# Napoliee/Expressive-FastSpeech2-Mandarin

Measured on AMD Instinct MI355X. Metric: mel-frames/sec/GPU (batch-64 synth) at 1/2/4/8 MI355X; RTF, higher is better.
Workload: dtype bf16; 1 GPU; cfg2: batch=64 x 64 phonemes per GPU, ESD-Chinese-Singing-MFA model.yaml, FastSpeech2.forward eval bf16; global_batch=64, seq_len=64, mel_frames_per_gpu_batch=24883, T_max=430, parallelism=dp1 (independent shards, no collective), hip_graph=True

## Files before the change

expressive-fastspeech2-mandarin_amd/csrc/wconv.hip:

```cpp
#include <type_traits>
#include <utility>

#include "conv_common.h"
#include "fs2_common.h"

namespace {

constexpr int kUnitB = 4096;

struct WconvArgs {
  const bf16 *x;
  int64_t xs;
  const bf16 *w;
  const float *bias;
  bf16 *out;
  int64_t os;
  int B, T, M, pad;
  uint32_t x_bytes, w_bytes;
  const int2 *row_pos;
  const int32_t *rows_dev;
  int out_sc1;
  const bf16 *w2;
  const float *bias2;
  const float *res;
  int64_t rs;
  float *out2;
  int64_t os2;
// ... 372 lines not shown
#pragma unroll 2
  for (int i = tid; i < BM * CPR; i += NT) {
    const int m = i / CPR, ch = i - m * CPR;
    if (m0 + m < M)
      store16_out(ob, (uint32_t)(m0 + m) * orow + (uint32_t)ch * 16u,
                  *reinterpret_cast<const uint4 *>(smem + X_OFF + m * OPITCH + ch * 16), p.out_sc1);
  }
  }
}


struct PnHeadArgs {
  const bf16 *x;
  int64_t xs;
  const bf16 *w1, *w2;
  const float *b1, *b2;
  bf16 *out;
  int64_t os;
  int T, M, pad;
  uint32_t x_bytes, w1_bytes, w2_bytes;
  const int2 *row_pos;
  const int32_t *rows_dev;
  int out_sc1;
};

__global__ __launch_bounds__(512, 1) void pn_head_kernel(PnHeadArgs p) {
  constexpr int KS = 5, CIN1 = 80, NCOL = 512, MB = 7, BM = 112, NWV = 8, NT = 512, JB = 4, DEPTH = 4;
  constexpr int YR = BM + KS - 1;
  constexpr int XR = BM + 2 * (KS - 1);
  constexpr int YPITCH = NCOL * 2 + 32;
  constexpr int XPITCH = CIN1 * 2 + 16;
  constexpr int OPITCH = NCOL * 2 + 16;
  constexpr int XPIECES = (XR * XPITCH + 1023) / 1024;
  constexpr int XPW = (XPIECES + NWV - 1) / NWV;
  constexpr int NU1 = (KS * CIN1 + 31) / 32;
  constexpr int NKS = NCOL / 32;
  constexpr int NU2 = KS * NKS;
  constexpr int ZBYTES = NKS * 64;
  constexpr int Y_OFF = ZBYTES;
  constexpr int YREG = YR * YPITCH > BM * OPITCH ? YR * YPITCH : BM * OPITCH;
  constexpr int X_OFF = Y_OFF + YREG;
  constexpr int B1_OFF = X_OFF + NWV * XPW * 1024;
  constexpr int B2_OFF = B1_OFF + NCOL * 4;
  constexpr int SMEM = B2_OFF + NCOL * 4;
  static_assert(SMEM <= 163840, "LDS");
  __shared__ __attribute__((aligned(16))) char smem[SMEM];

  const int tid = threadIdx.x, lane = tid & 63;
  const int w = __builtin_amdgcn_readfirstlane(tid >> 6);
  const int M = p.rows_dev != nullptr ? min(*p.rows_dev, p.M) : p.M, T = p.T, pad = p.pad;
  const int m0 = blockIdx.x * BM;
  if (m0 >= M) return;
  const int hrow0 = lane & 15, hi = lane >> 4;
  auto taps = [&](int gm) {
    int v = 0;
    if (gm >= 0 && gm < M) {
      int tpos, tlen;
      seq_pos(p.row_pos, gm, T, tpos, tlen);
#pragma unroll
      for (int tap = 0; tap < KS; ++tap) v |= ((unsigned)(tpos + tap - pad) < (unsigned)tlen ? 1 : 0) << tap;
    }
    return v;
  };
  for (int i = tid; i < ZBYTES / 16; i += NT) *reinterpret_cast<float4 *>(smem + 16 * i) = make_float4(0.f, 0.f, 0.f, 0.f);
  if (w < 4)
    __builtin_amdgcn_raw_ptr_buffer_load_lds(make_rsrc(w < 2 ? p.b1 : p.b2, NCOL * 4),
                                             (__attribute__((address_space(3))) void *)(smem + B1_OFF + w * 1024), 16,
                                             (uint32_t)((w & 1) * 1024 + lane * 16), 0, 0, 0);

  const rsrc_t xr = make_rsrc(p.x, p.x_bytes);
  const rsrc_t w1r = make_rsrc(p.w1, p.w1_bytes), w2r = make_rsrc(p.w2, p.w2_bytes);
  const uint32_t xrow = (uint32_t)p.xs * 2u;
#pragma unroll
  for (int i = 0; i < XPW; ++i) {
    const int pc = w + NWV * i;
    const int o = pc * 1024 + lane * 16;
    const int r = o / XPITCH, within = o - r * XPITCH;
    const int gm = m0 - 2 * pad + r;
    const bool ok = r < XR && within < CIN1 * 2 && gm >= 0 && gm < M;
    __builtin_amdgcn_raw_ptr_buffer_load_lds(xr, (__attribute__((address_space(3))) void *)(smem + X_OFF + pc * 1024),
                                             16, ok ? (uint32_t)gm * xrow + (uint32_t)within : kOOB, 0, 0, 0);
  }

  const uint32_t lane_off = (uint32_t)lane * 16u;
  const uint32_t wb1 = (uint32_t)(w * NU1) * (uint32_t)kUnitB, wb2 = (uint32_t)(w * NU2) * (uint32_t)kUnitB;
  bf16x8 pa[DEPTH][JB];
  auto load_at = [&](auto S, int u) {
    constexpr int s = decltype(S)::value;
    const bool c1 = u < 2 * NU1;
    const int uu = c1 ? (u < NU1 ? u : u - NU1) : (u - 2 * NU1 < NU2 ? u - 2 * NU1 : 0);
    const rsrc_t r = c1 ? w1r : w2r;
    const uint32_t so = (c1 ? wb1 : wb2) + (uint32_t)uu * (uint32_t)kUnitB;
    __builtin_amdgcn_sched_barrier(0);
#pragma unroll
    for (int jb = 0; jb < JB; ++jb)
      pa[s][jb] = __builtin_bit_cast(bf16x8, __builtin_amdgcn_raw_buffer_load_b128(r, lane_off + jb * 1024, so, 0));
    __builtin_amdgcn_sched_barrier(0);
  };
  static_for<DEPTH>([&](auto S) { load_at(S, decltype(S)::value); });
  asm volatile("s_waitcnt vmcnt(%0)" ::"n"(4 * DEPTH) : "memory");
  __builtin_amdgcn_s_waitcnt(kLgkm0);
  __syncthreads();

  static_for<2>([&](auto PASS) {
    constexpr int ps = decltype(PASS)::value;
    int vm1[4];
#pragma unroll
    for (int mb = 0; mb < 4; ++mb) vm1[mb] = taps(m0 - pad + (4 * ps + mb) * 16 + hrow0);
    f32x4 acc[JB][4];
#pragma unroll
    for (int i = 0; i < JB; ++i)
#pragma unroll
      for (int j = 0; j < 4; ++j) acc[i][j] = f32x4{0.f, 0.f, 0.f, 0.f};
    auto bases = [&](int u, int (&ad)[4]) {
      const int k = 32 * u + 8 * hi;
      const int tap = k / CIN1, c = k - tap * CIN1;
      const int base = X_OFF + ((4 * ps) * 16 + hrow0 + tap) * XPITCH + c * 2;
#pragma unroll
      for (int mb = 0; mb < 4; ++mb)
        ad[mb] = tap < KS ? (base + mb * 16 * XPITCH) & __builtin_amdgcn_sbfe(vm1[mb], tap, 1) : 0;
    };
    bf16x8 f0[4], f1[4];
    auto rd = [&](const int (&ad)[4], bf16x8 (&f)[4]) {
#pragma unroll
      for (int mb = 0; mb < 4; ++mb) f[mb] = *reinterpret_cast<const bf16x8 *>(smem + ad[mb]);
// ... 17 lines not shown
#pragma unroll
    for (int jb = 0; jb < JB; ++jb) {
      const int n = w * 64 + jb * 16 + 4 * hi;
      const float4 bb = *reinterpret_cast<const float4 *>(smem + B1_OFF + 4 * n);
#pragma unroll
      for (int mb = 0; mb < 4; ++mb) {
        const int r = (4 * ps + mb) * 16 + hrow0;
        const f32x4 v = acc[jb][mb];
        bf16x4 o;
        o[0] = (bf16)tanh_fast(v[0] + bb.x);
        o[1] = (bf16)tanh_fast(v[1] + bb.y);
        o[2] = (bf16)tanh_fast(v[2] + bb.z);
        o[3] = (bf16)tanh_fast(v[3] + bb.w);
        if (r < YR) *reinterpret_cast<bf16x4 *>(smem + Y_OFF + r * YPITCH + n * 2) = o;
      }
    }
  });
  __builtin_amdgcn_s_waitcnt(kLgkm0);
  __syncthreads();

  int vm2[MB];
#pragma unroll
  for (int mb = 0; mb < MB; ++mb) vm2[mb] = taps(m0 + mb * 16 + hrow0);
  auto bases_x = [&](int tap, int (&ad)[MB]) {
    const int base = Y_OFF + (hrow0 + tap) * YPITCH + hi * 16;
#pragma unroll
    for (int mb = 0; mb < MB; ++mb) ad[mb] = (base + mb * 16 * YPITCH) & __builtin_amdgcn_sbfe(vm2[mb], tap, 1);
  };
  bf16x8 f0[MB], f1[MB];
  auto issue_x = [&](const int (&ad)[MB], auto KSI, bf16x8 (&f)[MB]) {
    constexpr int off = decltype(KSI)::value * 64;
#pragma unroll
    for (int mb = 0; mb < MB; ++mb) f[mb] = *reinterpret_cast<const bf16x8 *>(smem + ad[mb] + off);
  };
  f32x4 acc[JB][MB];
#pragma unroll
  for (int i = 0; i < JB; ++i)
#pragma unroll
    for (int j = 0; j < MB; ++j) acc[i][j] = f32x4{0.f, 0.f, 0.f, 0.f};
  auto mma = [&](const bf16x8 (&fa)[JB], const bf16x8 (&fb)[MB]) {
#pragma unroll
    for (int mb = 0; mb < MB; ++mb)
#pragma unroll
      for (int jb = 0; jb < JB; ++jb)
        acc[jb][mb] = __builtin_amdgcn_mfma_f32_16x16x32_bf16(fa[jb], fb[mb], acc[jb][mb], 0, 0, 0);
  };
  constexpr int S0 = 2 * NU1;
  int bxc[MB], bxn[MB];
  bases_x(0, bxc);
  issue_x(bxc, std::integral_constant<int, 0>{}, f0);
#pragma nounroll
  for (int tap = 0; tap < KS; ++tap) {
    bases_x(tap + 1, bxn);
    static_for<NKS>([&](auto KSI) {
      constexpr int ks = decltype(KSI)::value, sl = (S0 + ks) % DEPTH;
      if constexpr (ks + 1 < NKS) {
        if constexpr (ks & 1)
          issue_x(bxc, std::integral_constant<int, ks + 1>{}, f0);
        else
          issue_x(bxc, std::integral_constant<int, ks + 1>{}, f1);
      } else {
        issue_x(bxn, std::integral_constant<int, 0>{}, f0);
      }
      if constexpr (ks & 1)
        mma(pa[sl], f1);
      else
        mma(pa[sl], f0);
      load_at(std::integral_constant<int, sl>{}, S0 + tap * NKS + ks + DEPTH);
    });
#pragma unroll
    for (int mb = 0; mb < MB; ++mb) bxc[mb] = bxn[mb];
  }

  asm volatile("s_waitcnt vmcnt(0)" ::: "memory");
  __builtin_amdgcn_s_waitcnt(kLgkm0);
  __syncthreads();
#pragma unroll
  for (int nb = 0; nb < JB; ++nb) {
    const int n = w * 64 + nb * 16 + 4 * hi;
    const float4 bb = *reinterpret_cast<const float4 *>(smem + B2_OFF + 4 * n);
#pragma unroll
    for (int mb = 0; mb < MB; ++mb) {
      const f32x4 v = acc[nb][mb];
      bf16x4 o;
      o[0] = (bf16)tanh_fast(v[0] + bb.x);
      o[1] = (bf16)tanh_fast(v[1] + bb.y);
      o[2] = (bf16)tanh_fast(v[2] + bb.z);
      o[3] = (bf16)tanh_fast(v[3] + bb.w);
      *reinterpret_cast<bf16x4 *>(smem + Y_OFF + (hrow0 + mb * 16) * OPITCH + n * 2) = o;
    }
  }
  __syncthreads();
  constexpr int CPR = NCOL * 2 / 16;
  char *ob = reinterpret_cast<char *>(p.out);
  const uint32_t orow = (uint32_t)p.os * 2u;
#pragma unroll 2
  for (int i = tid; i < BM * CPR; i += NT) {
    const int m = i / CPR, ch = i - m * CPR;
    if (m0 + m < M)
      store16_out(ob, (uint32_t)(m0 + m) * orow + (uint32_t)ch * 16u,
                  *reinterpret_cast<const uint4 *>(smem + Y_OFF + m * OPITCH + ch * 16), p.out_sc1);
  }
}


struct PnTailArgs {
  const bf16 *x;
  int64_t xs;
  const bf16 *w;
  const float *bias;
  const float *res;
  int64_t rs;
  float *out;
  int64_t os;
  int T, M, pad;
  uint32_t x_bytes, w_bytes;
  const int2 *row_pos;
  const int32_t *rows_dev;
};

__global__ __launch_bounds__(256, 1) void pn_tail_kernel(PnTailArgs p) {
  constexpr int KS = 5, CIN = 512, NB = 5, NCOL = 80, BM = 112, NST = 3, KPS = 2;
  constexpr int XR = BM + KS - 1;
// ... 221 lines not shown
    p.w2_bytes = (uint32_t)(fs2_wconv_weight_elems(5, 512, 80) * 2);
    hipLaunchKernelGGL((wconv_kernel<5, 512, 1, true>), dim3((unsigned)((Mg + 107) / 108)), dim3(512), 0,
                       as_stream(stream), p);
  } else if (d->w2 != nullptr) {
    if (d->Cin != 80 || d->bias2 == nullptr || d->pad != 2) return FS2_EUNSUPPORTED;
    PnHeadArgs q;
    q.x = p.x;
    q.xs = p.xs;
    q.w1 = p.w;
    q.w2 = reinterpret_cast<const bf16 *>(d->w2);
    q.b1 = d->bias;
    q.b2 = d->bias2;
    q.out = p.out;
    q.os = p.os;
    q.T = p.T;
    q.M = p.M;
    q.pad = p.pad;
    q.x_bytes = p.x_bytes;
    q.w1_bytes = p.w_bytes;
    q.w2_bytes = (uint32_t)(fs2_wconv_weight_elems(d->KS, 512, 512) * 2);
    q.row_pos = row_pos;
    q.rows_dev = d->rows_dev;
    q.out_sc1 = env_out_sc1();
    hipLaunchKernelGGL(pn_head_kernel, dim3(nwg), dim3(512), 0, as_stream(stream), q);
  } else if (d->Cin == 80)
    hipLaunchKernelGGL((wconv_kernel<5, 80, 1>), dim3(nwg), dim3(512), 0, as_stream(stream), p);
  else
    hipLaunchKernelGGL((wconv_kernel<5, 512, WCONV_WQ>), dim3(nwg), dim3(512 / WCONV_WQ), 0, as_stream(stream), p);
  FS2_CHECK_LAUNCH();
  return FS2_OK;
}
```

expressive-fastspeech2-mandarin_amd/fs2amd/_lib.py:

```python
import ctypes
import os

import torch

HERE = os.path.dirname(os.path.abspath(__file__))
DEFAULT_LIB = os.path.join(HERE, "_lib", "libfs2hip.so")

FS2_F32, FS2_BF16, FS2_FP8 = 0, 1, 2
FS2_I16 = 3
FS2_F64 = 4
PITCH_T_MAX, PITCH_T_MAX_NOFILL, OUTLIER_LDS_BYTES = 131072, 4096, 65536
F0_GROUP, F0_LDS_BYTES = 8, 65536
RESAMPLE_LDS_BYTES = 81920
MAS_LDS_BYTES, MAS_LDS_SMALL, FORWARD_SUM_LDS_BYTES = 163840, 32768, 65536
MAS_AUTO, MAS_LDS, MAS_GLOBAL = 0, 1, 2
ALIGN_SIZE_CAP = 1 << 24
DTW_LDS_BYTES, DTW_LDS_SMALL = 163840, 32768
DTW_AUTO, DTW_LDS, DTW_GLOBAL = 0, 1, 2
EVAL_SIZE_CAP = 1 << 24
F0_TRACK_THR, F0_TRACK_CAP_MAX, F0_TRACK_BINS_MAX, F0_TRACK_STEP_MAX, F0_TRACK_TB = 100, 101, 256, 63, 64
F0_TRACK_LDS_BYTES = 65536
VAD_SUMS_BYTES, VAD_AREA_BYTES, VAD_TILE_FRAMES, VAD_CHUNK_FRAMES, VAD_B_MAX = 32768, 32768, 192, 256, 65535
PVOC_BLOCK, PVOC_J_CAP, PVOC_B_MAX = 64, 2 ** 31 - 1, 65535
IIR_BLOCK, IIR_CHUNK, IIR_S_MAX, IIR_TABLE_LEN, IIR_B_MAX, LOUD_H_MAX = 64, 16384, 8, 412, 65535, 32768
# ... 63 lines not shown
        ("group_n", _i), ("group_cin", _i),
    ]


class Ffn8Desc(ctypes.Structure):

    _fields_ = [
        ("x8", _p), ("x8_row_stride", _i64), ("res", _p), ("res_row_stride", _i64), ("w", _p),
        ("cs1", _p), ("b1", _p), ("inv_sf", _f), ("cs2", _p), ("b2", _p),
        ("B", _i), ("T", _i), ("D", _i), ("F", _i), ("KS", _i), ("pad", _i),
        ("ln_gamma", _p), ("ln_beta", _p), ("ln_eps", _f),
        ("out", _p), ("out_row_stride", _i64), ("out8", _p), ("out8_row_stride", _i64), ("out8_scale", _f),
        ("rows_dev", _p), ("row_pos", _p), ("rows_max", _i),
    ]


class WconvDesc(ctypes.Structure):

    _fields_ = [
        ("x", _p), ("x_row_stride", _i64), ("w", _p), ("bias", _p),
        ("B", _i), ("T", _i), ("Cin", _i), ("N", _i), ("KS", _i), ("pad", _i), ("epilogue", _i),
        ("out", _p), ("out_row_stride", _i64), ("w2", _p), ("bias2", _p), ("residual", _p), ("res_row_stride", _i64),
        ("rows_dev", _p), ("row_pos", _p), ("rows_max", _i),
    ]


class CondDesc(ctypes.Structure):

    _fields_ = [
        ("speakers", _p), ("speaker_table", _p), ("n_speaker", _i), ("emotions", _p), ("emo_table", _p),
        ("n_emo", _i), ("d_emo", _i), ("arousals", _p), ("aro_table", _p), ("n_aro", _i), ("d_aro", _i),
        ("valences", _p), ("val_table", _p), ("n_val", _i), ("d_val", _i), ("lin_w", _p), ("lin_b", _p),
        ("spk_out", _p), ("emo_out", _p),
    ]


class CondGrads(ctypes.Structure):

    _fields_ = [("d_speaker_table", _p), ("d_emo_table", _p), ("d_aro_table", _p), ("d_val_table", _p),
                ("d_lin_w", _p), ("d_lin_b", _p)]


class FfnDesc(ctypes.Structure):

    _fields_ = [
        ("x", _p), ("x_row_stride", _i64),
# ... 282 lines not shown
    "fs2_f0_track_lds_bytes": (_i64, [_i, _i]),
    "fs2_f0_track_workspace_bytes": (_i64, [_i, _i, _i, _i, _i]),
    "fs2_f0_track": (_i, [_p, _p, _i, _i, _i, _d, _i, _i, _d, _d, _p, _p, _p, _p, _p, _i, _p, _p, _i, _d, _d, _p, _i64,
                          _p, _p, _p, _p]),
}


SIGNATURES_VAD = {
    "fs2_vad_frames": (_i64, [_i64, _i64]),
    "fs2_vad_workspace_bytes": (_i64, [_i64, _i64, _i64, _i64]),
    "fs2_vad_lds_bytes": (_i64, [_i64, _i64]),
    "fs2_vad_power": (_i, [_p, _i, _i64, _p, _i, _i, _i, _i, _p, _p, _p, _i64, _p]),
    "fs2_vad_intervals": (_i, [_p, _p, _p, _i, _i, _i, _d, _d, _i, _i64, _i, _i, _p, _p, _p, _p, _p]),
    "fs2_vad_cut": (_i, [_p, _i, _i64, _p, _i, _i, _i, _p, _p, _p]),
}


SIGNATURES_PVOC = {
    "fs2_pvoc_frames": (_i64, [_i64, _d]),
    "fs2_phase_vocoder": (_i, [ctypes.POINTER(PvocDesc), _p]),
}


SIGNATURES_IIR = {
    "fs2_iir_blocks": (_i64, [_i64]),
    "fs2_iir_chunks": (_i64, [_i64]),
    "fs2_loudness_blocks": (_i64, [_i64, _i64]),
    "fs2_loudness_workspace_bytes": (_i64, [_i64, _i64, _i64]),
    "fs2_sosfilt": (_i, [_p, _i, _i64, _p, _i, _i, _p, _p, _i, _p, _p, _p, _p, _p]),
    "fs2_loudness_gate": (_i, [_p, _p, _i, _i, _i, _d, _d, _p, _p, _p, _i64, _p]),
    "fs2_gain_int16": (_i, [_p, _i, _i64, _p, _i, _i, _p, _d, _d, _p, _p, _p, _p, _p, _p]),
}


def iir_blocks(n):
    return 0 if n < 1 else (n - 1) // IIR_BLOCK + 1


def iir_chunks(n):
    return 0 if n < 1 else (n - 1) // IIR_CHUNK + 1


def loudness_blocks(n, H):
    return 0 if n < 1 or n < 4 * H else (n - 4 * H) // H + 1


# ... 121 lines not shown

def header_symbols(header_path):
    import re

    text = open(header_path).read()
    return sorted(set(re.findall(r"\b(fs2_[a-z0-9_]+)\s*\(", text)) - {"fs2_conv_desc"})


_LIB = None
CSRC = os.path.join(os.path.dirname(HERE), "csrc")
HEADER = os.path.join(os.path.dirname(os.path.dirname(HERE)), "include", "fs2hip.h")
HEADER_PROSODY = os.path.join(os.path.dirname(HEADER), "fs2hip_prosody.h")
HEADER_AUDIO = os.path.join(os.path.dirname(HEADER), "fs2hip_audio.h")
HEADER_AUDIO_INV = os.path.join(os.path.dirname(HEADER), "fs2hip_audio_inv.h")
HEADER_PREP = os.path.join(os.path.dirname(HEADER), "fs2hip_prep.h")
HEADER_F0 = os.path.join(os.path.dirname(HEADER), "fs2hip_f0.h")
HEADER_RESAMPLE = os.path.join(os.path.dirname(HEADER), "fs2hip_resample.h")
HEADER_ALIGN = os.path.join(os.path.dirname(HEADER), "fs2hip_align.h")
HEADER_EVAL = os.path.join(os.path.dirname(HEADER), "fs2hip_eval.h")
HEADER_F0_TRACK = os.path.join(os.path.dirname(HEADER), "fs2hip_f0_track.h")
HEADER_VAD = os.path.join(os.path.dirname(HEADER), "fs2hip_vad.h")
HEADER_PVOC = os.path.join(os.path.dirname(HEADER), "fs2hip_pvoc.h")
HEADER_IIR = os.path.join(os.path.dirname(HEADER), "fs2hip_iir.h")
EXTRA_HEADERS = ("fs2hip_prosody.h", "fs2hip_audio.h", "fs2hip_audio_inv.h", "fs2hip_prep.h", "fs2hip_f0.h",
                 "fs2hip_resample.h", "fs2hip_align.h", "fs2hip_eval.h", "fs2hip_f0_track.h", "fs2hip_vad.h",
                 "fs2hip_pvoc.h", "fs2hip_iir.h")


def source_build_id(csrc=CSRC, header=HEADER):
    import hashlib

    if not os.path.isdir(csrc) or not os.path.exists(header):
        return None
    h = hashlib.sha256()
    for name in sorted(f for f in os.listdir(csrc) if f.endswith((".hip", ".h"))):
        h.update(name.encode())
        with open(os.path.join(csrc, name), "rb") as f:
            h.update(f.read())
    with open(header, "rb") as f:
        h.update(b"fs2hip.h")
        h.update(f.read())
    for name in EXTRA_HEADERS:
        with open(os.path.join(os.path.dirname(header), name), "rb") as f:
            h.update(name.encode())
            h.update(f.read())
    return h.hexdigest()[:16]


def lib_path():
    return os.environ.get("FS2_LIB", DEFAULT_LIB)


def load():
    global _LIB
    if _LIB is not None:
        return _LIB
    path = lib_path()
    if not os.path.exists(path):
        raise RuntimeError(
            f"fs2amd: HIP library not found at {path}. Build it with `python -c 'import __graft_entry__ as g; "
            f"g.build()'` (hipcc --offload-arch=gfx950). There is no CPU fallback.")
    lib = ctypes.CDLL(path, mode=ctypes.RTLD_GLOBAL)
    allow_missing = "FS2_LIB" in os.environ and os.environ.get("FS2_LIB_ALLOW_MISSING") == "1"
    for name, (res, args) in list(SIGNATURES.items()) + list(SIGNATURES_PROSODY.items()) + \
            list(SIGNATURES_AUDIO.items()) + list(SIGNATURES_AUDIO_INV.items()) + list(SIGNATURES_PREP.items()) + \
            list(SIGNATURES_F0.items()) + list(SIGNATURES_RESAMPLE.items()) + list(SIGNATURES_ALIGN.items()) + \
            list(SIGNATURES_EVAL.items()) + list(SIGNATURES_F0_TRACK.items()) + list(SIGNATURES_VAD.items()) + \
            list(SIGNATURES_PVOC.items()) + list(SIGNATURES_IIR.items()):
        if allow_missing and not hasattr(lib, name):
            continue
        fn = getattr(lib, name)
        fn.restype = res
        fn.argtypes = args
    if "FS2_LIB" not in os.environ:
        want = source_build_id()
        got = lib.fs2_build_id().decode()
        if want is not None and got != want:
            raise RuntimeError(f"fs2amd: {path} was built from other sources (fs2_build_id {got}, sources "
                               f"{want}); rebuild with `python -c 'import __graft_entry__ as g; g.build()'`")
    _LIB = lib
    return lib


def check(rc, what):
    if rc != FS2_OK:
        msg = load().fs2_status_string(rc).decode()
        raise RuntimeError(f"{what} failed: fs2 status {rc} ({msg})")
```

expressive-fastspeech2-mandarin_amd/fs2amd/ops.py:

```python
import collections
import ctypes
import os

import torch

from . import _lib as L

_lib = L.load()


def _ptr(t):
    return None if t is None else ctypes.c_void_p(t.data_ptr())


def _stream(t):
    return ctypes.c_void_p(torch.cuda.current_stream(t.device).cuda_stream)


def _dt(t):
    if t.dtype == torch.bfloat16:
        return L.FS2_BF16
    if t.dtype == torch.float32:
        return L.FS2_F32
    if t.dtype == torch.float8_e4m3fn:
# ... 409 lines not shown
            out = torch.empty(*rs, 80, device=x.device, dtype=torch.float32)
        d = L.WconvDesc()
        _wconv_layout(d, layout)
        d.x, d.x_row_stride = x.data_ptr(), _rows(x, "x")
        d.w, d.bias = w_packed.data_ptr(), bias.data_ptr()
        d.B, d.T, d.Cin, d.N, d.KS, d.pad, d.epilogue = B, T, cin, N, ks, pad, L.EPI_BIAS_TANH
        d.out, d.out_row_stride = out.data_ptr(), _rows(out, "out")
        d.w2, d.bias2 = wt.data_ptr(), bt.data_ptr()
        d.residual, d.res_row_stride = res.data_ptr(), _rows(res, "residual")
        L.check(_lib.fs2_wconv(ctypes.byref(d), _stream(x)), "fs2_wconv")
        return out
    if out is None:
        out = torch.empty(*rs, N, device=x.device, dtype=torch.bfloat16)
    d = L.WconvDesc()
    _wconv_layout(d, layout)
    d.x, d.x_row_stride = x.data_ptr(), _rows(x, "x")
    d.w, d.bias = w_packed.data_ptr(), bias.data_ptr()
    d.B, d.T, d.Cin, d.N, d.KS, d.pad, d.epilogue = B, T, cin, N, ks, pad, L.EPI_BIAS_TANH
    d.out, d.out_row_stride = out.data_ptr(), _rows(out, "out")
    if second is not None:
        d.w2, d.bias2 = second[0].data_ptr(), second[1].data_ptr()
    L.check(_lib.fs2_wconv(ctypes.byref(d), _stream(x)), "fs2_wconv")
    return out


FFN_SLOTS = 256


def ffn_part_bytes(tile_rows):
    return 4 * 4 * (tile_rows // 16) * 64 * 16


def rows_bucket(rows, capacity, step=1024):
    return min(capacity, -(-int(rows) // step) * step)


FFN_COST = {112: (20.0, 10.0, {1: 0.0, 2: 10.0, 4: 16.0}), 96: (17.5, 8.5, {2: 10.0}),
            64: (13.0, 5.0, {1: 0.0, 2: 9.0, 4: 21.0})}


def ffn_form(rows, F):
    nch = F // 256
    if not _splitk_on[0]:
        return 112, 1
    best = None
    for tr, (chunk, base, over) in FFN_COST.items():
# ... 1989 lines not shown
```

expressive-fastspeech2-mandarin_amd/fs2amd/runtime.py:

```python
import os
from types import SimpleNamespace

import numpy as np
import torch

from . import _lib as L
from . import ops
from .model import sinusoid_table


def _mask(lengths, width):
    if lengths.is_cuda:
        return ops.length_mask(lengths, width)
    ids = torch.arange(0, width, device=lengths.device).unsqueeze(0).expand(lengths.shape[0], -1)
    return ids >= lengths.unsqueeze(1).expand(-1, width)


def _pe(P, which, n):
    tab = P.enc_pe if which == "enc" else P.dec_pe
    if n <= tab.shape[0]:
        return tab
    key = f"_pe_{which}_{n}"
    if not hasattr(P, key):
        setattr(P, key, sinusoid_table(n, tab.shape[1]).to(tab.device))
# ... 468 lines not shown
    dec_lens = st.mel_len if g.d_targets is None else g.mel_lens
    frame_level = not (st.phoneme_p and st.phoneme_e)
    x = st.x
    if not frame_level and T_dec == T_out and packed_decoder_ok(P):
        x, lay = decode_packed(P, st, x, dec_lens, T_out, rows_hint)
        mel, pn = mel_postnet(P, x, lay, dec_lens, postnet_valid, rows_hint)
        return mel, pn, st
    _ensure_lr(st)
    if frame_level:
        x = ops.lr_expand(x, st.cum, st.mel_len, T_out, pe=None, out_dtype=P.act_dtype)
        if not st.phoneme_p:
            st.p_pred = _variance(P, "pitch", x, dec_lens, g.p_targets, p_control)
        if not st.phoneme_e:
            st.e_pred = _variance(P, "energy", x, dec_lens, g.e_targets, e_control)
        x = x[:, :T_dec].contiguous()
        x = _add_pe(x, _pe(P, "dec", T_dec))
    else:
        x = ops.lr_expand(x, st.cum, st.mel_len, T_out, pe=_pe(P, "dec", T_out), out_dtype=P.act_dtype)
        if T_dec != T_out:
            x = x[:, :T_dec].contiguous()
    if T_dec != T_out:
        dec_lens = torch.clamp(dec_lens, max=T_dec)
    x = _stack(P, P.dec_layers, x, dec_lens, timed=True)
    mel_bf = _mel_copy(P, x, x.shape[:2])
    mel = ops.conv1d(x, P.mel_w, P.mel_b, cin=P.d_model, ks=1, pad=0, compute=P.compute, epilogue=L.EPI_BIAS,
                     out_dtype=L.FS2_F32, out2=mel_bf)
    return mel, _postnet(P, mel, mel_bf, dec_lens if postnet_valid else None, rows_hint), st


def decode_packed(P, st, x, dec_lens, T_lay, rows_hint=None):
    x, lay, qkv0 = _lr_packed(P, st, x, dec_lens, T_lay, rows_hint)
    return _stack(P, P.dec_layers, x, None, layout=lay, timed=True, qkv0=qkv0), lay


def decode_packed_head(P, st, x, dec_lens, T_lay, rows_hint=None):
    x, lay, qkv0 = _lr_packed(P, st, x, dec_lens, T_lay, rows_hint)
    x1, qkv1 = _stack(P, P.dec_layers[:1], x, None, layout=lay, timed=True, qkv0=qkv0, tail_next=P.dec_layers[1])
    return x1, lay, qkv1


def decode_packed_rest(P, x1, lay, qkv1):
    return _stack(P, P.dec_layers[1:], x1, None, layout=lay, timed=True, qkv0=qkv1)


def _lr_packed(P, st, x, dec_lens, T_lay, rows_hint=None):
    qkv0 = None
# ... 16 lines not shown
            qkv0 = r[-1] if proj is not None else None
    else:
        _ensure_lr(st)
        lay = ops.SeqLayout(dec_lens, T_lay)
        x = ops.lr_expand(x, st.cum, st.mel_len, T_lay, pe=_pe(P, "dec", T_lay), out_dtype=P.act_dtype,
                          out_layout=lay)
    lay.rows_hint = None if rows_hint is None else ops.rows_bucket(rows_hint, lay.capacity)
    return x, lay, qkv0


def phoneme_qkv0(P, x):
    lp = P.dec_layers[0]
    with _Timed("dec:qkv0"):
        return ops.conv1d(x, lp.wqkv, None, cin=x.shape[-1], ks=1, pad=0, compute=P.compute, epilogue=L.EPI_BIAS,
                          out_dtype=L.FS2_F32)


def split_stage2_ok(P):
    return (os.environ.get("FS2_SYNTH_SPLIT", "0") == "1" and len(P.dec_layers) >= 2
            and all(lp.fp8 is None for lp in P.dec_layers))


def mel_postnet(P, x, lay, dec_lens, postnet_valid=False, rows_hint=None):
    mel_bf = _mel_copy(P, x, (lay.B, lay.T))
    with _Timed("dec:mel"):
        mel = ops.conv1d(x, P.mel_w, P.mel_b, cin=P.d_model, ks=1, pad=0, compute=P.compute, epilogue=L.EPI_BIAS,
                         out_dtype=L.FS2_F32, src_layout=lay, out2=mel_bf)
    with _Timed("dec:postnet"):
        pn = _postnet(P, mel, mel_bf, dec_lens if postnet_valid else None, rows_hint)
    return mel, pn


def packed_stage2_ok(P, st, x):
    return st.phoneme_p and st.phoneme_e and packed_decoder_ok(P) and lr_fused_ok(x)


def run_forward(model, speakers, emotions, arousals, valences, texts, src_lens, max_src_len, mels, mel_lens,
                max_mel_len, p_targets, e_targets, d_targets, p_control, e_control, d_control):
    dev = texts.device
    if not _device_ok(dev):
        raise RuntimeError("fs2amd: FastSpeech2.forward runs on the HIP kernels only; move the model and the batch "
                           "to a ROCm device (no CPU fallback)")
    P = model.packed(dev)
    va = model.variance_adaptor
    ids = lambda t: None if t is None else torch.as_tensor(t).to(device=dev, dtype=torch.int64).contiguous()
    f32 = lambda t: None if t is None else t.to(device=dev, dtype=torch.float32).contiguous()
# ... 126 lines not shown

def _mel_copy_on(P):
    return P.compute == L.FS2_BF16 and os.environ.get("FS2_MEL_BF16", "1") != "0"


def _mel_copy(P, x, bt):
    if not _mel_copy_on(P):
        return None
    return torch.empty(*bt, P.mel_w.shape[0], device=x.device, dtype=torch.bfloat16)


POSTNET_REACH = 10
POSTNET_MARGIN = 2 * POSTNET_REACH


def wconv_on():
    return os.environ.get("FS2_WCONV", "1") != "0"


def pn_head_on():
    return os.environ.get("FS2_PN_HEAD", "1") != "0"


def pn_tail_fused_on():
    return os.environ.get("FS2_PN_TAIL_FUSED", "1") != "0"


def postnet_valid_region_on():
    return os.environ.get("FS2_POSTNET_VALID", "1") != "0"


def _postnet_consts(P, bf16_input):
    ent = getattr(P, "_postnet_consts", None)
    if ent is None:
        if torch.cuda.is_current_stream_capturing():
            raise RuntimeError("PostNet constants must be computed before graph capture (run the forward once)")
        b = P.mel_b.float().reshape(1, 1, -1).expand(1, 2 * POSTNET_MARGIN, -1).contiguous()
        y = _postnet(P, b, b.to(torch.bfloat16) if bf16_input else None)
        ent = (y[0, POSTNET_MARGIN].clone(), y[0, 2 * POSTNET_MARGIN - POSTNET_REACH:].clone())
        P._postnet_consts = ent
    return ent


def _postnet(P, mel, mel_bf=None, mel_len=None, sum_len=None):
    if mel_len is not None and postnet_valid_region_on() and mel.shape[0] > 0:
        return _postnet_valid(P, mel, mel_bf, mel_len, sum_len)
    y = mel if mel_bf is None else mel_bf
    return _postnet_convs(P, y, mel)


def _postnet_convs(P, y, res, layout=None):
    n_pn = len(P.postnet)
    first = 0
    if n_pn > 2 and y.dtype == torch.bfloat16 and wconv_on() and pn_head_on() and \
            getattr(P.postnet[0], "wfr", None) is not None and getattr(P.postnet[1], "wfr", None) is not None and \
            P.postnet[0].cin == 80 and P.postnet[0].k == 5 and P.postnet[0].p == 2 and P.postnet[1].p == 2:
        l0, l1 = P.postnet[0], P.postnet[1]
        y = ops.wconv(y, l0.wfr, l0.b, ks=l0.k, pad=l0.p, second=(l1.wfr, l1.b), layout=layout)
        first = 2
    last = P.postnet[-1]
    for i, lp in enumerate(P.postnet):
        if i < first:
            continue
        if i == n_pn - 2 and n_pn > 2 and getattr(lp, "wfr", None) is not None and lp.cin == 512 and lp.k == 5 \
                and lp.p == 2 and getattr(last, "wtail", None) is not None and last.cin == 512 and last.k == 5 \
                and last.p == 2 and wconv_on() and pn_tail_fused_on() \
                and y.dtype == torch.bfloat16 and res.dtype == torch.float32:
            return ops.wconv(y, lp.wfr, lp.b, ks=lp.k, pad=lp.p, layout=layout,
                             tail=(last.wtail, last.b, res.contiguous()))
        if i < n_pn - 1 and getattr(lp, "wfr", None) is not None and wconv_on() and y.dtype == torch.bfloat16:
            y = ops.wconv(y, lp.wfr, lp.b, ks=lp.k, pad=lp.p, layout=layout)
        elif i < n_pn - 1:
            y = ops.conv1d(y, lp.w, lp.b, cin=lp.cin, ks=lp.k, pad=lp.p, compute=P.compute,
                           epilogue=L.EPI_BIAS_TANH, out_dtype=P.act_dtype, layout=layout)
        elif getattr(lp, "wtail", None) is not None and wconv_on() and y.dtype == torch.bfloat16 \
                and res.dtype == torch.float32:
            y = ops.wconv_tail(y, lp.wtail, lp.b, res.contiguous(), ks=lp.k, pad=lp.p, layout=layout)
# ... 25 lines not shown
```

Before: 18.64 million mel-frames/s.

## Fuse mel projection and first three postnet convs into one HIP kernel

Adds a templated variant of the postnet head kernel. It computes the 256→80 mel linear projection from decoder rows in LDS, then runs postnet conv 0 (80→512), conv 1 and conv 2 (512→512) back to back inside one workgroup. Each 112-row block produces 108 output rows and recomputes a halo so the third conv can stay on-chip. This removes a separate mel projection launch and the global-memory round trip of one 512-wide intermediate activation. The cost is redundant halo rows, a longer kernel with heavier LDS reuse, and use only when the valid-region postnet path is off.

```diff
diff --git a/expressive-fastspeech2-mandarin_amd/csrc/wconv.hip b/expressive-fastspeech2-mandarin_amd/csrc/wconv.hip
--- a/expressive-fastspeech2-mandarin_amd/csrc/wconv.hip
+++ b/expressive-fastspeech2-mandarin_amd/csrc/wconv.hip
@@ -3,6 +3,7 @@
 
 #include "conv_common.h"
 #include "fs2_common.h"
+#include "fs2hip_postnet.h"
 
 namespace {
 
@@ -421,10 +422,24 @@
   const int2 *row_pos;
   const int32_t *rows_dev;
   int out_sc1;
+  const bf16 *dx;
+  int64_t dxs;
+  uint32_t dx_bytes;
+  const int32_t *rowmap;
+  const bf16 *wm;
+  const float *bm;
+  float *mel;
+  int64_t mels;
+  bf16 *mel_bf;
+  const bf16 *w3;
+  const float *b3;
 };
 
+template <bool H3>
 __global__ __launch_bounds__(512, 1) void pn_head_kernel(PnHeadArgs p) {
   constexpr int KS = 5, CIN1 = 80, NCOL = 512, MB = 7, BM = 112, NWV = 8, NT = 512, JB = 4, DEPTH = 4;
+  constexpr int TB = H3 ? BM - (KS - 1) : BM;
+  constexpr int RO = H3 ? (KS - 1) / 2 : 0;
   constexpr int YR = BM + KS - 1;
   constexpr int XR = BM + 2 * (KS - 1);
   constexpr int YPITCH = NCOL * 2 + 32;
@@ -441,34 +456,75 @@
   constexpr int X_OFF = Y_OFF + YREG;
   constexpr int B1_OFF = X_OFF + NWV * XPW * 1024;
   constexpr int B2_OFF = B1_OFF + NCOL * 4;
-  constexpr int SMEM = B2_OFF + NCOL * 4;
+  constexpr int B3_OFF = B2_OFF + NCOL * 4;
+  constexpr int DK = 256, NM = 80, DPITCH = DK * 2 + 16, DPW = 8, WMPW = 6;
+  constexpr int WM_OFF = Y_OFF + NWV * DPW * 1024;
+  constexpr int BM_OFF = B3_OFF + NCOL * 4;
+  static_assert(XR * DPITCH <= NWV * DPW * 1024 && NM * DPITCH <= NWV * WMPW * 1024, "prologue pieces");
+  static_assert(WM_OFF + NWV * WMPW * 1024 <= Y_OFF + YREG && 128 * DPITCH <= YREG, "prologue fits the y1 region");
+  constexpr int SMEM = H3 ? BM_OFF + NM * 4 : B2_OFF + NCOL * 4;
   static_assert(SMEM <= 163840, "LDS");
   __shared__ __attribute__((aligned(16))) char smem[SMEM];
 
   const int tid = threadIdx.x, lane = tid & 63;
   const int w = __builtin_amdgcn_readfirstlane(tid >> 6);
-  const int M = p.rows_dev != nullptr ? min(*p.rows_dev, p.M) : p.M, T = p.T, pad = p.pad;
-  const int m0 = blockIdx.x * BM;
-  if (m0 >= M) return;
+  const int M = !H3 && p.rows_dev != nullptr ? min(*p.rows_dev, p.M) : p.M, T = p.T, pad = p.pad;
+  if ((int)blockIdx.x * TB >= M) return;
+  const int m0 = (int)blockIdx.x * TB - RO;
   const int hrow0 = lane & 15, hi = lane >> 4;
   auto taps = [&](int gm) {
     int v = 0;
     if (gm >= 0 && gm < M) {
       int tpos, tlen;
-      seq_pos(p.row_pos, gm, T, tpos, tlen);
+      seq_pos(H3 ? nullptr : p.row_pos, gm, T, tpos, tlen);
 #pragma unroll
       for (int tap = 0; tap < KS; ++tap) v |= ((unsigned)(tpos + tap - pad) < (unsigned)tlen ? 1 : 0) << tap;
     }
     return v;
   };
   for (int i = tid; i < ZBYTES / 16; i += NT) *reinterpret_cast<float4 *>(smem + 16 * i) = make_float4(0.f, 0.f, 0.f, 0.f);
-  if (w < 4)
-    __builtin_amdgcn_raw_ptr_buffer_load_lds(make_rsrc(w < 2 ? p.b1 : p.b2, NCOL * 4),
+  if (w < (H3 ? 6 : 4))
+    __builtin_amdgcn_raw_ptr_buffer_load_lds(make_rsrc(w < 2 ? p.b1 : (w < 4 ? p.b2 : p.b3), NCOL * 4),
                                              (__attribute__((address_space(3))) void *)(smem + B1_OFF + w * 1024), 16,
                                              (uint32_t)((w & 1) * 1024 + lane * 16), 0, 0, 0);
 
+  const rsrc_t w1r = make_rsrc(p.w1, p.w1_bytes), w2r = make_rsrc(p.w2, p.w2_bytes);
+  const rsrc_t w3r = make_rsrc(H3 ? p.w3 : p.w2, p.w2_bytes);
+  if constexpr (H3) {
+    if (w == 7 && lane < NM / 4)
+      *reinterpret_cast<float4 *>(smem + BM_OFF + 16 * lane) = reinterpret_cast<const float4 *>(p.bm)[lane];
+    for (int i = tid; i < (NWV * XPW * 1024 - XR * XPITCH) / 16; i += NT)
+      *reinterpret_cast<float4 *>(smem + X_OFF + XR * XPITCH + 16 * i) = make_float4(0.f, 0.f, 0.f, 0.f);
+    int src[DPW];
+#pragma unroll
+    for (int i = 0; i < DPW; ++i) {
+      const int r = ((w + NWV * i) * 1024 + lane * 16) / DPITCH;
+      const int gm = m0 - 2 * pad + r;
+      src[i] = -1;
+      if (r < XR && gm >= 0 && gm < M) src[i] = p.rowmap != nullptr ? p.rowmap[gm] : gm;
+    }
+    const rsrc_t wmr = make_rsrc(p.wm, NM * DK * 2), dr = make_rsrc(p.dx, p.dx_bytes);
+#pragma unroll
+    for (int i = 0; i < WMPW; ++i) {
+      const int pc = w + NWV * i;
+      const int o = pc * 1024 + lane * 16;
+      const int r = o / DPITCH, within = o - r * DPITCH;
+      const bool ok = r < NM && within < DK * 2;
+      __builtin_amdgcn_raw_ptr_buffer_load_lds(wmr, (__attribute__((address_space(3))) void *)(smem + WM_OFF + pc * 1024),
+                                               16, ok ? (uint32_t)(r * DK * 2 + within) : kOOB, 0, 0, 0);
+    }
+    const uint32_t drow = (uint32_t)p.dxs * 2u;
+#pragma unroll
+    for (int i = 0; i < DPW; ++i) {
+      const int pc = w + NWV * i;
+      const int o = pc * 1024 + lane * 16;
+      const int within = o - (o / DPITCH) * DPITCH;
+      const bool ok = src[i] >= 0 && within < DK * 2;
+      __builtin_amdgcn_raw_ptr_buffer_load_lds(dr, (__attribute__((address_space(3))) void *)(smem + Y_OFF + pc * 1024),
+                                               16, ok ? (uint32_t)src[i] * drow + (uint32_t)within : kOOB, 0, 0, 0);
+    }
+  } else {
   const rsrc_t xr = make_rsrc(p.x, p.x_bytes);
-  const rsrc_t w1r = make_rsrc(p.w1, p.w1_bytes), w2r = make_rsrc(p.w2, p.w2_bytes);
   const uint32_t xrow = (uint32_t)p.xs * 2u;
 #pragma unroll
   for (int i = 0; i < XPW; ++i) {
@@ -480,26 +536,65 @@
     __builtin_amdgcn_raw_ptr_buffer_load_lds(xr, (__attribute__((address_space(3))) void *)(smem + X_OFF + pc * 1024),
                                              16, ok ? (uint32_t)gm * xrow + (uint32_t)within : kOOB, 0, 0, 0);
   }
+  }
 
   const uint32_t lane_off = (uint32_t)lane * 16u;
   const uint32_t wb1 = (uint32_t)(w * NU1) * (uint32_t)kUnitB, wb2 = (uint32_t)(w * NU2) * (uint32_t)kUnitB;
   bf16x8 pa[DEPTH][JB];
   auto load_at = [&](auto S, int u) {
     constexpr int s = decltype(S)::value;
-    const bool c1 = u < 2 * NU1;
-    const int uu = c1 ? (u < NU1 ? u : u - NU1) : (u - 2 * NU1 < NU2 ? u - 2 * NU1 : 0);
-    const rsrc_t r = c1 ? w1r : w2r;
+    const bool c1 = u < 2 * NU1, c2 = !H3 || u < 2 * NU1 + NU2;
+    const int u2 = c2 ? u - 2 * NU1 : u - 2 * NU1 - NU2;
+    const int uu = c1 ? (u < NU1 ? u : u - NU1) : (u2 < NU2 ? u2 : 0);
+    const rsrc_t r = c1 ? w1r : (c2 ? w2r : w3r);
     const uint32_t so = (c1 ? wb1 : wb2) + (uint32_t)uu * (uint32_t)kUnitB;
     __builtin_amdgcn_sched_barrier(0);
 #pragma unroll
     for (int jb = 0; jb < JB; ++jb)
-      pa[s][jb] = __builtin_bit_cast(bf16x8, __builtin_amdgcn_raw_buffer_load_b128(r, lane_off + jb * 1024, so, 0));
+      if constexpr (H3)
+        pa[s][jb] = __builtin_bit_cast(bf16x8, __builtin_amdgcn_raw_buffer_load_b128(r, lane_off, so + jb * 1024, 0));
+      else
+        pa[s][jb] = __builtin_bit_cast(bf16x8, __builtin_amdgcn_raw_buffer_load_b128(r, lane_off + jb * 1024, so, 0));
     __builtin_amdgcn_sched_barrier(0);
   };
   static_for<DEPTH>([&](auto S) { load_at(S, decltype(S)::value); });
   asm volatile("s_waitcnt vmcnt(%0)" ::"n"(4 * DEPTH) : "memory");
   __builtin_amdgcn_s_waitcnt(kLgkm0);
   __syncthreads();
+
+  if constexpr (H3) {
+    f32x4 am[NM / 16];
+#pragma unroll
+    for (int nb = 0; nb < NM / 16; ++nb) am[nb] = f32x4{0.f, 0.f, 0.f, 0.f};
+    const char *ab = smem + Y_OFF + (16 * w + hrow0) * DPITCH + hi * 16;
+    const char *bb = smem + WM_OFF + hrow0 * DPITCH + hi * 16;
+#pragma unroll
+    for (int s = 0; s < DK / 32; ++s) {
+      const bf16x8 fa = *reinterpret_cast<const bf16x8 *>(ab + s * 64);
+#pragma unroll
+      for (int nb = 0; nb < NM / 16; ++nb)
+        am[nb] = __builtin_amdgcn_mfma_f32_16x16x32_bf16(
+            fa, *reinterpret_cast<const bf16x8 *>(bb + nb * 16 * DPITCH + s * 64), am[nb], 0, 0, 0);
+    }
+#pragma unroll
+    for (int nb = 0; nb < NM / 16; ++nb) {
+      const int n = nb * 16 + hrow0;
+      const float bn = *reinterpret_cast<const float *>(smem + BM_OFF + 4 * n);
+#pragma unroll
+      for (int v = 0; v < 4; ++v) {
+        const int r = 16 * w + 4 * hi + v, gm = m0 - 2 * pad + r;
+        const bool in = gm >= 0 && gm < M;
+        const float y = am[nb][v] + bn;
+        if (r < XR) *reinterpret_cast<bf16 *>(smem + X_OFF + r * XPITCH + n * 2) = in ? (bf16)y : (bf16)0.0f;
+        if (in && r >= 2 * pad + RO && r < 2 * pad + RO + TB) {
+          p.mel[(size_t)gm * p.mels + n] = y;
+          if (p.mel_bf != nullptr) p.mel_bf[(size_t)gm * NM + n] = (bf16)y;
+        }
+      }
+    }
+    __builtin_amdgcn_s_waitcnt(kLgkm0);
+    __syncthreads();
+  }
 
   static_for<2>([&](auto PASS) {
     constexpr int ps = decltype(PASS)::value;
@@ -563,8 +658,9 @@
   int vm2[MB];
 #pragma unroll
   for (int mb = 0; mb < MB; ++mb) vm2[mb] = taps(m0 + mb * 16 + hrow0);
+  int lbase = Y_OFF + hrow0 * YPITCH + hi * 16;
   auto bases_x = [&](int tap, int (&ad)[MB]) {
-    const int base = Y_OFF + (hrow0 + tap) * YPITCH + hi * 16;
+    const int base = lbase + tap * YPITCH;
 #pragma unroll
     for (int mb = 0; mb < MB; ++mb) ad[mb] = (base + mb * 16 * YPITCH) & __builtin_amdgcn_sbfe(vm2[mb], tap, 1);
   };
@@ -575,10 +671,6 @@
     for (int mb = 0; mb < MB; ++mb) f[mb] = *reinterpret_cast<const bf16x8 *>(smem + ad[mb] + off);
   };
   f32x4 acc[JB][MB];
-#pragma unroll
-  for (int i = 0; i < JB; ++i)
-#pragma unroll
-    for (int j = 0; j < MB; ++j) acc[i][j] = f32x4{0.f, 0.f, 0.f, 0.f};
   auto mma = [&](const bf16x8 (&fa)[JB], const bf16x8 (&fb)[MB]) {
 #pragma unroll
     for (int mb = 0; mb < MB; ++mb)
@@ -586,13 +678,18 @@
       for (int jb = 0; jb < JB; ++jb)
         acc[jb][mb] = __builtin_amdgcn_mfma_f32_16x16x32_bf16(fa[jb], fb[mb], acc[jb][mb], 0, 0, 0);
   };
-  constexpr int S0 = 2 * NU1;
+  auto conv512 = [&](auto S0C) {
+  constexpr int S0 = decltype(S0C)::value;
+#pragma unroll
+  for (int i = 0; i < JB; ++i)
+#pragma unroll
+    for (int j = 0; j < MB; ++j) acc[i][j] = f32x4{0.f, 0.f, 0.f, 0.f};
   int bxc[MB], bxn[MB];
   bases_x(0, bxc);
   issue_x(bxc, std::integral_constant<int, 0>{}, f0);
 #pragma nounroll
   for (int tap = 0; tap < KS; ++tap) {
-    bases_x(tap + 1, bxn);
+    if constexpr (!H3) bases_x(tap + 1, bxn);
     static_for<NKS>([&](auto KSI) {
       constexpr int ks = decltype(KSI)::value, sl = (S0 + ks) % DEPTH;
       if constexpr (ks + 1 < NKS) {
@@ -601,6 +698,7 @@
         else
           issue_x(bxc, std::integral_constant<int, ks + 1>{}, f1);
       } else {
+        if constexpr (H3) bases_x(tap + 1, bxn);
         issue_x(bxn, std::integral_constant<int, 0>{}, f0);
       }
       if constexpr (ks & 1)
@@ -612,14 +710,46 @@
 #pragma unroll
     for (int mb = 0; mb < MB; ++mb) bxc[mb] = bxn[mb];
   }
+  };
+  conv512(std::integral_constant<int, 2 * NU1>{});
+  int tE = tid;
+  if constexpr (H3) {
+    __builtin_amdgcn_s_waitcnt(kLgkm0);
+    __syncthreads();
+    asm volatile("" : "+v"(tE));
+    const int hrow0 = tE & 15, hi = (tE & 63) >> 4;
+#pragma unroll
+    for (int nb = 0; nb < JB; ++nb) {
+      const int n = w * 64 + nb * 16 + 4 * hi;
+      const float4 bb = *reinterpret_cast<const float4 *>(smem + B2_OFF + 4 * n);
+#pragma unroll
+      for (int mb = 0; mb < MB; ++mb) {
+        const f32x4 v = acc[nb][mb];
+        bf16x4 o;
+        o[0] = (bf16)tanh_fast(v[0] + bb.x);
+        o[1] = (bf16)tanh_fast(v[1] + bb.y);
+        o[2] = (bf16)tanh_fast(v[2] + bb.z);
+        o[3] = (bf16)tanh_fast(v[3] + bb.w);
+        *reinterpret_cast<bf16x4 *>(smem + Y_OFF + (hrow0 + mb * 16) * YPITCH + n * 2) = o;
+      }
+    }
+#pragma unroll
+    for (int mb = 0; mb < MB; ++mb) vm2[mb] = mb * 16 + hrow0 < TB ? taps(m0 + RO + mb * 16 + hrow0) : 0;
+    lbase = Y_OFF + hrow0 * YPITCH + hi * 16;
+    __builtin_amdgcn_s_waitcnt(kLgkm0);
+    __syncthreads();
+    conv512(std::integral_constant<int, 2 * NU1 + NU2>{});
+    asm volatile("" : "+v"(tE));
+  }
 
   asm volatile("s_waitcnt vmcnt(0)" ::: "memory");
   __builtin_amdgcn_s_waitcnt(kLgkm0);
   __syncthreads();
+  const int hrE = tE & 15, hiE = (tE & 63) >> 4;
 #pragma unroll
   for (int nb = 0; nb < JB; ++nb) {
-    const int n = w * 64 + nb * 16 + 4 * hi;
-    const float4 bb = *reinterpret_cast<const float4 *>(smem + B2_OFF + 4 * n);
+    const int n = w * 64 + nb * 16 + 4 * hiE;
+    const float4 bb = *reinterpret_cast<const float4 *>(smem + (H3 ? B3_OFF : B2_OFF) + 4 * n);
 #pragma unroll
     for (int mb = 0; mb < MB; ++mb) {
       const f32x4 v = acc[nb][mb];
@@ -628,7 +758,7 @@
       o[1] = (bf16)tanh_fast(v[1] + bb.y);
       o[2] = (bf16)tanh_fast(v[2] + bb.z);
       o[3] = (bf16)tanh_fast(v[3] + bb.w);
-      *reinterpret_cast<bf16x4 *>(smem + Y_OFF + (hrow0 + mb * 16) * OPITCH + n * 2) = o;
+      *reinterpret_cast<bf16x4 *>(smem + Y_OFF + (hrE + mb * 16) * OPITCH + n * 2) = o;
     }
   }
   __syncthreads();
@@ -636,10 +766,10 @@
   char *ob = reinterpret_cast<char *>(p.out);
   const uint32_t orow = (uint32_t)p.os * 2u;
 #pragma unroll 2
-  for (int i = tid; i < BM * CPR; i += NT) {
+  for (int i = tE; i < BM * CPR; i += NT) {
     const int m = i / CPR, ch = i - m * CPR;
-    if (m0 + m < M)
-      store16_out(ob, (uint32_t)(m0 + m) * orow + (uint32_t)ch * 16u,
+    if (m < TB && m0 + RO + m < M)
+      store16_out(ob, (uint32_t)(m0 + RO + m) * orow + (uint32_t)ch * 16u,
                   *reinterpret_cast<const uint4 *>(smem + Y_OFF + m * OPITCH + ch * 16), p.out_sc1);
   }
 }
@@ -907,7 +1037,7 @@
     q.row_pos = row_pos;
     q.rows_dev = d->rows_dev;
     q.out_sc1 = env_out_sc1();
-    hipLaunchKernelGGL(pn_head_kernel, dim3(nwg), dim3(512), 0, as_stream(stream), q);
+    hipLaunchKernelGGL(pn_head_kernel<false>, dim3(nwg), dim3(512), 0, as_stream(stream), q);
   } else if (d->Cin == 80)
     hipLaunchKernelGGL((wconv_kernel<5, 80, 1>), dim3(nwg), dim3(512), 0, as_stream(stream), p);
   else
@@ -915,3 +1045,51 @@
   FS2_CHECK_LAUNCH();
   return FS2_OK;
 }
+
+extern "C" int fs2_pn_head3(const fs2_pn_head3_desc *d, fs2_stream_t stream) {
+  if (d == nullptr || d->x == nullptr || d->mel_w == nullptr || d->mel_b == nullptr || d->mel == nullptr ||
+      d->out == nullptr)
+    return FS2_EINVAL;
+  for (int i = 0; i < 3; ++i)
+    if (d->w[i] == nullptr || d->bias[i] == nullptr) return FS2_EINVAL;
+  if (d->B < 0 || d->T < 0 || d->x_rows < 0 || d->x_row_stride < 256 || (d->x_row_stride & 7) ||
+      d->mel_row_stride < 80 || d->out_row_stride < 512 || (d->out_row_stride & 7))
+    return FS2_EINVAL;
+  const int64_t M64 = (int64_t)d->B * d->T;
+  if (M64 == 0) return FS2_OK;
+  if (d->rowmap == nullptr && d->x_rows < M64) return FS2_EINVAL;
+  const int64_t xb = d->x_rows * d->x_row_stride * 2, ob = M64 * d->out_row_stride * 2;
+  if (xb >= (1LL << 31) || ob >= (1LL << 32) || M64 > 0x7fffff00LL) return FS2_EUNSUPPORTED;
+  PnHeadArgs q;
+  q.x = nullptr;
+  q.xs = 0;
+  q.x_bytes = 0;
+  q.w1 = reinterpret_cast<const bf16 *>(d->w[0]);
+  q.w2 = reinterpret_cast<const bf16 *>(d->w[1]);
+  q.w3 = reinterpret_cast<const bf16 *>(d->w[2]);
+  q.b1 = d->bias[0];
+  q.b2 = d->bias[1];
+  q.b3 = d->bias[2];
+  q.out = reinterpret_cast<bf16 *>(d->out);
+  q.os = d->out_row_stride;
+  q.T = d->T;
+  q.M = (int)M64;
+  q.pad = 2;
+  q.w1_bytes = (uint32_t)(fs2_wconv_weight_elems(5, 80, 512) * 2);
+  q.w2_bytes = (uint32_t)(fs2_wconv_weight_elems(5, 512, 512) * 2);
+  q.row_pos = nullptr;
+  q.rows_dev = nullptr;
+  q.out_sc1 = env_out_sc1();
+  q.dx = reinterpret_cast<const bf16 *>(d->x);
+  q.dxs = d->x_row_stride;
+  q.dx_bytes = (uint32_t)xb;
+  q.rowmap = d->rowmap;
+  q.wm = reinterpret_cast<const bf16 *>(d->mel_w);
+  q.bm = d->mel_b;
+  q.mel = d->mel;
+  q.mels = d->mel_row_stride;
+  q.mel_bf = reinterpret_cast<bf16 *>(d->mel_bf16);
+  hipLaunchKernelGGL(pn_head_kernel<true>, dim3((unsigned)((M64 + 107) / 108)), dim3(512), 0, as_stream(stream), q);
+  FS2_CHECK_LAUNCH();
+  return FS2_OK;
+}
diff --git a/expressive-fastspeech2-mandarin_amd/fs2amd/_lib.py b/expressive-fastspeech2-mandarin_amd/fs2amd/_lib.py
--- a/expressive-fastspeech2-mandarin_amd/fs2amd/_lib.py
+++ b/expressive-fastspeech2-mandarin_amd/fs2amd/_lib.py
@@ -109,6 +109,15 @@
         ("B", _i), ("T", _i), ("Cin", _i), ("N", _i), ("KS", _i), ("pad", _i), ("epilogue", _i),
         ("out", _p), ("out_row_stride", _i64), ("w2", _p), ("bias2", _p), ("residual", _p), ("res_row_stride", _i64),
         ("rows_dev", _p), ("row_pos", _p), ("rows_max", _i),
+    ]
+
+
+class PnHead3Desc(ctypes.Structure):
+
+    _fields_ = [
+        ("x", _p), ("x_row_stride", _i64), ("x_rows", _i64), ("rowmap", _p), ("mel_w", _p), ("mel_b", _p),
+        ("mel", _p), ("mel_row_stride", _i64), ("mel_bf16", _p), ("w", _p * 3), ("bias", _p * 3),
+        ("B", _i), ("T", _i), ("out", _p), ("out_row_stride", _i64),
     ]
 
 
@@ -437,6 +446,10 @@
 }
 
 
+SIGNATURES_POSTNET = {
+    "fs2_pn_head3": (_i, [ctypes.POINTER(PnHead3Desc), _p]),
+}
+
 SIGNATURES_IIR = {
     "fs2_iir_blocks": (_i64, [_i64]),
     "fs2_iir_chunks": (_i64, [_i64]),
@@ -604,9 +617,10 @@
 HEADER_VAD = os.path.join(os.path.dirname(HEADER), "fs2hip_vad.h")
 HEADER_PVOC = os.path.join(os.path.dirname(HEADER), "fs2hip_pvoc.h")
 HEADER_IIR = os.path.join(os.path.dirname(HEADER), "fs2hip_iir.h")
+HEADER_POSTNET = os.path.join(os.path.dirname(HEADER), "fs2hip_postnet.h")
 EXTRA_HEADERS = ("fs2hip_prosody.h", "fs2hip_audio.h", "fs2hip_audio_inv.h", "fs2hip_prep.h", "fs2hip_f0.h",
                  "fs2hip_resample.h", "fs2hip_align.h", "fs2hip_eval.h", "fs2hip_f0_track.h", "fs2hip_vad.h",
-                 "fs2hip_pvoc.h", "fs2hip_iir.h")
+                 "fs2hip_pvoc.h", "fs2hip_iir.h", "fs2hip_postnet.h")
 
 
 def source_build_id(csrc=CSRC, header=HEADER):
@@ -648,7 +662,7 @@
             list(SIGNATURES_AUDIO.items()) + list(SIGNATURES_AUDIO_INV.items()) + list(SIGNATURES_PREP.items()) + \
             list(SIGNATURES_F0.items()) + list(SIGNATURES_RESAMPLE.items()) + list(SIGNATURES_ALIGN.items()) + \
             list(SIGNATURES_EVAL.items()) + list(SIGNATURES_F0_TRACK.items()) + list(SIGNATURES_VAD.items()) + \
-            list(SIGNATURES_PVOC.items()) + list(SIGNATURES_IIR.items()):
+            list(SIGNATURES_PVOC.items()) + list(SIGNATURES_IIR.items()) + list(SIGNATURES_POSTNET.items()):
         if allow_missing and not hasattr(lib, name):
             continue
         fn = getattr(lib, name)
diff --git a/expressive-fastspeech2-mandarin_amd/fs2amd/ops.py b/expressive-fastspeech2-mandarin_amd/fs2amd/ops.py
--- a/expressive-fastspeech2-mandarin_amd/fs2amd/ops.py
+++ b/expressive-fastspeech2-mandarin_amd/fs2amd/ops.py
@@ -455,6 +455,39 @@
         d.w2, d.bias2 = second[0].data_ptr(), second[1].data_ptr()
     L.check(_lib.fs2_wconv(ctypes.byref(d), _stream(x)), "fs2_wconv")
     return out
+
+
+def pn_head3(x, mel_w, mel_b, convs, B, T, *, src_layout=None, mel_bf=None):
+    (w0, b0), (w1, b1), (w2, b2) = convs
+    _gpu(x, mel_w, mel_b, w0, b0, w1, b1, w2, b2)
+    if x.dtype != torch.bfloat16 or mel_w.dtype != torch.bfloat16 or any(w.dtype != torch.bfloat16 for w in (w0, w1, w2)):
+        raise TypeError("fs2amd.pn_head3: bf16 activations and weights only")
+    x2 = x if x.dim() == 2 else x.reshape(-1, x.shape[-1])
+    assert x2.shape[1] == 256 and mel_w.is_contiguous() and mel_w.numel() == 80 * 256 and mel_b.numel() == 80
+    assert w0.numel() == _lib.fs2_wconv_weight_elems(5, 80, 512) and b0.numel() == 512
+    assert all(w.numel() == _lib.fs2_wconv_weight_elems(5, 512, 512) and b.numel() == 512 for w, b in ((w1, b1), (w2, b2)))
+    assert all(w.is_contiguous() for w in (w0, w1, w2))
+    if src_layout is not None:
+        assert (src_layout.B, src_layout.T) == (B, T) and x2.shape[0] >= src_layout.capacity
+    else:
+        assert x2.shape[0] == B * T
+    mel = torch.empty(B, T, 80, device=x.device, dtype=torch.float32)
+    out = torch.empty(B, T, 512, device=x.device, dtype=torch.bfloat16)
+    d = L.PnHead3Desc()
+    d.x, d.x_row_stride, d.x_rows = x2.data_ptr(), _rows(x2, "x"), x2.shape[0]
+    if src_layout is not None:
+        d.rowmap = src_layout.rowmap.data_ptr()
+    d.mel_w, d.mel_b = mel_w.data_ptr(), mel_b.data_ptr()
+    d.mel, d.mel_row_stride = mel.data_ptr(), 80
+    if mel_bf is not None:
+        assert mel_bf.dtype == torch.bfloat16 and mel_bf.is_contiguous() and tuple(mel_bf.shape) == (B, T, 80)
+        d.mel_bf16 = mel_bf.data_ptr()
+    for i, (w, b) in enumerate(((w0, b0), (w1, b1), (w2, b2))):
+        d.w[i], d.bias[i] = w.data_ptr(), b.data_ptr()
+    d.B, d.T = B, T
+    d.out, d.out_row_stride = out.data_ptr(), 512
+    L.check(_lib.fs2_pn_head3(ctypes.byref(d), _stream(x)), "fs2_pn_head3")
+    return mel, out
 
 
 FFN_SLOTS = 256
diff --git a/expressive-fastspeech2-mandarin_amd/fs2amd/runtime.py b/expressive-fastspeech2-mandarin_amd/fs2amd/runtime.py
--- a/expressive-fastspeech2-mandarin_amd/fs2amd/runtime.py
+++ b/expressive-fastspeech2-mandarin_amd/fs2amd/runtime.py
@@ -514,6 +514,9 @@
     if T_dec != T_out:
         dec_lens = torch.clamp(dec_lens, max=T_dec)
     x = _stack(P, P.dec_layers, x, dec_lens, timed=True)
+    if pn_head3_ok(P, x, postnet_valid):
+        mel, y = _pn_head3(P, x, x.shape[0], x.shape[1])
+        return mel, _postnet_convs(P, y, mel, first=3), st
     mel_bf = _mel_copy(P, x, x.shape[:2])
     mel = ops.conv1d(x, P.mel_w, P.mel_b, cin=P.d_model, ks=1, pad=0, compute=P.compute, epilogue=L.EPI_BIAS,
                      out_dtype=L.FS2_F32, out2=mel_bf)
@@ -576,6 +579,10 @@
 
 
 def mel_postnet(P, x, lay, dec_lens, postnet_valid=False, rows_hint=None):
+    if pn_head3_ok(P, x, postnet_valid):
+        with _Timed("dec:postnet"):
+            mel, y = _pn_head3(P, x, lay.B, lay.T, lay)
+            return mel, _postnet_convs(P, y, mel, first=3)
     mel_bf = _mel_copy(P, x, (lay.B, lay.T))
     with _Timed("dec:mel"):
         mel = ops.conv1d(x, P.mel_w, P.mel_b, cin=P.d_model, ks=1, pad=0, compute=P.compute, epilogue=L.EPI_BIAS,
@@ -748,6 +755,22 @@
     return os.environ.get("FS2_PN_HEAD", "1") != "0"
 
 
+def pn_head3_on():
+    return os.environ.get("FS2_PN_HEAD3", "1") != "0"
+
+
+def pn_head3_ok(P, x, postnet_valid=False):
+    pn = P.postnet
+    return (pn_head3_on() and pn_head_on() and wconv_on() and not postnet_valid and _mel_copy_on(P)
+            and x.dtype == torch.bfloat16 and x.shape[-1] == 256 and P.mel_w.numel() == 80 * 256 and len(pn) > 3
+            and all(getattr(l, "wfr", None) is not None and l.k == 5 and l.p == 2 for l in pn[:3])
+            and pn[0].cin == 80 and pn[1].cin == 512 and pn[2].cin == 512)
+
+
+def _pn_head3(P, x, B, T, lay=None):
+    return ops.pn_head3(x, P.mel_w, P.mel_b, [(l.wfr, l.b) for l in P.postnet[:3]], B, T, src_layout=lay)
+
+
 def pn_tail_fused_on():
     return os.environ.get("FS2_PN_TAIL_FUSED", "1") != "0"
 
@@ -775,10 +798,9 @@
     return _postnet_convs(P, y, mel)
 
 
-def _postnet_convs(P, y, res, layout=None):
+def _postnet_convs(P, y, res, layout=None, first=0):
     n_pn = len(P.postnet)
-    first = 0
-    if n_pn > 2 and y.dtype == torch.bfloat16 and wconv_on() and pn_head_on() and \
+    if first == 0 and n_pn > 2 and y.dtype == torch.bfloat16 and wconv_on() and pn_head_on() and \
             getattr(P.postnet[0], "wfr", None) is not None and getattr(P.postnet[1], "wfr", None) is not None and \
             P.postnet[0].cin == 80 and P.postnet[0].k == 5 and P.postnet[0].p == 2 and P.postnet[1].p == 2:
         l0, l1 = P.postnet[0], P.postnet[1]
diff --git a/include/fs2hip_postnet.h b/include/fs2hip_postnet.h
--- /dev/null
+++ b/include/fs2hip_postnet.h
@@ -0,0 +1,33 @@
+#ifndef FS2HIP_POSTNET_H
+#define FS2HIP_POSTNET_H
+
+#include "fs2hip.h"
+
+#ifdef __cplusplus
+extern "C" {
+#endif
+
+typedef struct fs2_pn_head3_desc {
+  const void *x;
+  int64_t x_row_stride;
+  int64_t x_rows;
+  const int32_t *rowmap;
+  const void *mel_w;
+  const float *mel_b;
+  float *mel;
+  int64_t mel_row_stride;
+  void *mel_bf16;
+  const void *w[3];
+  const float *bias[3];
+  int B, T;
+  void *out;
+  int64_t out_row_stride;
+} fs2_pn_head3_desc;
+
+int fs2_pn_head3(const fs2_pn_head3_desc *d, fs2_stream_t stream);
+
+#ifdef __cplusplus
+}
+#endif
+
+#endif
```

Result: faster. 18.92 million mel-frames/s, median of 6 (+1.5%).
